# claserken/SISS

Hardware: AMD Instinct MI355X
Metric: unlearning samples/sec (= unlearning-steps/sec x batch x gpus), CelebA-HQ-256 DDPM SISS (higher is better)
Workload: dtype bf16; 1 GPU; delete_celeb.yaml: CelebA-HQ 256x256 DDPM UNet (113.7M params), SISS lambd=0.5, t=999, bf16, bs=16/GPU, GA=1, scaling_norm=500, AdamW lr 5e-6; loss_fn=importance_sampling_with_mixture, global_batch=16, grad_accum=1, parallelism=dp1, hipgraph=True

## Files before the change

### include/siss_hip.h

```cpp
#ifndef SISS_HIP_H
#define SISS_HIP_H
#include <stdint.h>
#ifdef __cplusplus
extern "C" {
#endif

typedef struct siss_tn_job {
    const void* Y; long ldy; const void* X; long ldx; float* dW; long set_stride;
    int N, C, npanels, nsets, rows_per_set, row_begin, row_end, nsplits;
    long x_set_rows;
    const void* zero_page; float* dbias; float* dbias2;
    int shifts[9]; int coffs[9];
    long bias_set_stride;
} siss_tn_job;

typedef struct siss_rk_terms {
    const double* row[8]; double c[8]; int n;
} siss_rk_terms;

long siss_loss_partials_words(int B, long chw);
int siss_mixture_fwd(const void* x0, const void* a0, const void* noise, int in_bf16, const int64_t* t, const
    float* u, const float* alphas_cumprod, const float* gamma_tab, const float* sigma_tab, float lambd, int B,
    long chw, void* x_mix, float* gamma_t, float* sigma_t, float* dist_x, float* dist_a, float* iw_x, float* iw_a,
    double* partials, void* stream);
// ... 18 lines not shown
int siss_dispatch_reset(void);
int siss_gemm_nt_set_c3p_blocks(int n);
int siss_gemm_nt(const void* A, long lda, const void* W, void* C, long ldc, const float* bias, const float*
    rowbias, long ldrb, const void* R, long ldr, int M, int N, int Kp, int npanels, const int* shifts, const int*
    coffs, int rows_per_image, int Hp, int Wp, float alpha, int batch, long strideA, long strideW, long strideC,
    void* stream);
int siss_gemm_nt_alpha_cols(const void* A, long lda, const void* W, void* C, long ldc, const float* bias,
    const void* R, long ldr, int M, int N, int Kp, float alpha, int alpha_cols, void* stream);
int siss_gemm_nt_qstats(const void* A, long lda, const void* W, void* C, long ldc, const float* bias, const
    float* rowbias, long ldrb, const void* R, long ldr, int M, int N, int Kp, int npanels, const int* shifts,
    const int* coffs, int rows_per_image, int Hp, int Wp, float alpha, float* qstats, int* written, void* stream);
int siss_conv3x3_sc_takes(int M, int N, int Kp, int K2, int rows_per_image, int Wp, long lda, long ldc, long
    lda2);
int siss_conv3x3_sc(const void* A, long lda, const void* W, void* C, long ldc, const float* bias, const float*
    rowbias, long ldrb, const void* A2, long lda2, const void* W2, int K2, const float* bias2, int M, int N, int
    Kp, const int* shifts, const int* coffs, int rows_per_image, int Hp, int Wp, float* qstats, int* written,
    void* stream);
int siss_conv3x3_dgrad_sc_takes(int M, int N, int Kp, int Nx, int rows_per_image, int Wp, long lda, long ldc,
    long ldcx, long ldr);
int siss_conv3x3_dgrad_sc(const void* A, long lda, const void* W, void* C, long ldc, const void* R, long ldr,
    const void* Wx, void* Cx, long ldcx, int Nx, int M, int N, int Kp, const int* shifts, const int* coffs, int
    rows_per_image, int Hp, int Wp, void* stream);
int siss_gemm_nt_d2s(const void* A, long lda, const void* W, void* C, long ldc, const void* R, long ldr, int
    M, int N, int Kp, int npanels, const int* shifts, const int* coffs, int rows_per_image, int Hp, int Wp, int
    plane, void* stream);
int siss_gemm_nt_d2s_bias(const void* A, long lda, const void* W, void* C, long ldc, const float* bias, int M,
    int N, int Kp, int npanels, const int* shifts, const int* coffs, int rows_per_image, int Hp, int Wp, int
    plane, void* stream);
int siss_gemm_nt_d2s_phases(const void* A, long lda, const void* W, void* C, long ldc, const float* bias,
    const void* R, long ldr, int M, int N, int Kp, const int* phase_p0, const int* shifts, const int* coffs, int
    rows_per_image, int Hp, int Wp, void* stream);
int siss_gemm_nt_geglu_bwd(const void* A, long lda, const void* W, void* dh, const void* h, long rows_x, int
    M, int N, int Kp, void* stream);
int siss_gemm_nt_geglu_fwd(const void* A, long lda, const void* W, const float* bias, void* h, void* y, int M,
    int F, int Kp, void* stream);
long siss_conv_qstats_words(long M, int N);
int siss_gemm_nt_mulsub(const void* A, long lda, const void* W, void* C, long ldc, const void* R, long ldr,
    const float* rowsub, int M, int N, int Kp, float alpha, int batch, long strideA, long strideW, long strideC,
    void* stream);

int siss_gemm_tn(const void* Y, long ldy, const void* X, long ldx, float* dW, long set_stride, int N, int C,
    int npanels, const int* shifts, const int* coffs, int nsets, int rows_per_set, long x_set_rows, int row_begin,
    int row_end, int nsplits, const void* zero_page, float* dbias, float* dbias2, void* stream);
int siss_gemm_tn_bs(const void* Y, long ldy, const void* X, long ldx, float* dW, long set_stride, int N, int
    C, int npanels, const int* shifts, const int* coffs, int nsets, int rows_per_set, long x_set_rows, int
    row_begin, int row_end, int nsplits, const void* zero_page, float* dbias, float* dbias2, long bias_set_stride,
    void* stream);
long siss_gemm_tn_overwrite_log(long* out, long max_records);
int siss_gemm_tn_set_pair_cost(int permille);
int siss_gemm_tn_pair(const void* job3, const void* job1, int max_blocks, void* stream);
int siss_gemm_tn_grouped(const void* jobs, int njobs, void* stream);
int siss_gemm_tn_grouped_capped(const void* jobs, int njobs, int max_blocks, void* stream);

int siss_groupnorm_set_slab(int on);
long siss_gn_partial_words(int n, int H, int W, int C, int G);
int siss_quad_stats(const void* x, long ld, int M, int N, int rows_per_image, float* qs, void* stream);
int siss_groupnorm_fwd_qs(const void* x, const float* gamma, const float* beta, void* y, float* mean, float*
    rstd, float* partial, const float* qsA, int ca, const float* qsB, int N, int H, int W, int C, int G, float
    eps, int silu, int out_compact, int ldx, void* stream);
int siss_groupnorm_fwd_ld(const void* x, const float* gamma, const float* beta, void* y, float* mean, float*
    rstd, float* partial, int N, int H, int W, int C, int G, float eps, int silu, int out_compact, int ldx, void*
    stream);
int siss_groupnorm_fwd(const void* x, const float* gamma, const float* beta, void* y, float* mean, float*
    rstd, float* partial, int N, int H, int W, int C, int G, float eps, int silu, int out_compact, void* stream);
int siss_groupnorm_bwd_ld(const void* dy, const void* x, const float* gamma, const float* beta, const float*
    mean, const float* rstd, void* dx, const void* accum, const void* accum2, void* dx2, int split_c, int
    accumulate2, float* dgamma, float* dbeta, float* colsum, long colsum_ld, float* partial, int n2, int nx, int
    set_images, long set_stride, int H, int W, int C, int G, int silu, int dy_compact, int ldx, void* stream);
int siss_groupnorm_bwd_ld_s2d(const void* dy, const void* x, const float* gamma, const float* beta, const
    float* mean, const float* rstd, void* dx, const void* accum, const void* accum2, void* dx2, int split_c, int
    accumulate2, float* dgamma, float* dbeta, float* colsum, long colsum_ld, float* partial, int n2, int nx, int
    set_images, long set_stride, int H, int W, int C, int G, int silu, int dy_compact, int ldx, void* stream);
int siss_groupnorm_bwd(const void* dy, const void* x, const float* gamma, const float* beta, const float*
    mean, const float* rstd, void* dx, const void* accum, const void* accum2, void* dx2, int split_c, int
    accumulate2, float* dgamma, float* dbeta, float* colsum, long colsum_ld, float* partial, int n2, int nx, int
    set_images, long set_stride, int H, int W, int C, int G, int silu, int dy_compact, void* stream);
int siss_groupnorm_bwd_sc(const void* dy, const void* x, const float* gamma, const float* beta, const float*
    mean, const float* rstd, void* dx, const void* dout, long ldo, const void* wsc, int K, const void* accum2,
    void* dx2, int split_c, int accumulate2, float* dgamma, float* dbeta, float* colsum, float* partial, float*
    gconst, int n2, int nx, int set_images, long set_stride, int H, int W, int C, int G, int silu, int s2d, int
    ldx, void* stream);

int siss_conv_out_fprop(const void* x, const float* w, const float* bias, float* pred, int B, int H, int W,
    int C, int CO, void* stream);
int siss_conv_out_dgrad(const float* c, const float* w, void* dx, int N2, int H, int W, int C, int CO, void*
    stream);
int siss_conv_out_wgrad(const float* c, const void* x, float* dW, float* dbias, int nsets, int set_images, int
    nx, long set_stride_w, long set_stride_b, int H, int W, int C, int CO, void* stream);
int siss_conv_in_dgrad(const void* dh, long ld, const void* w, int kp, float* dx, int N, int Cin, int H, int
    W, int C0, void* stream);
int siss_conv_in_dgrad_f32(const void* dh, long ld, const void* w, int kp, float* dx, int N, int Cin, int H,
    int W, int C0, void* stream);

int siss_softmax_fwd(const void* s, void* p, long rows, int S, void* stream);
int siss_softmax_bwd(const void* p, const void* dp, void* ds, long rows, long p_rows, int S, float scale,
    void* stream);
int siss_mha_small_takes(int S, int D, int training);
int siss_mha_small_fwd(const void* q, const void* k, const void* v, void* o, float* lse, int N, int S, int C,
    int D, float scale, void* stream);
int siss_mha_small_bwd(const void* q, const void* k, const void* v, const void* o, const float* lse, const
    void* dout, void* dq, void* dk, void* dv, int n2, int nx, int S, int C, int D, float scale, void* stream);
int siss_mha_small_fwd_f32(const void* q, const void* k, const void* v, void* o, float* lse, int N, int S, int
    C, int D, float scale, void* stream);
int siss_mha_small_bwd_f32(const void* q, const void* k, const void* v, const void* o, const float* lse, const
    void* dout, void* dq, void* dk, void* dv, int n2, int nx, int S, int C, int D, float scale, void* stream);

// ... 337 lines not shown
```

### siss_amd/csrc/common.h

```cpp
#pragma once
#include <hip/hip_runtime.h>
#include <stdint.h>

typedef uint16_t bf16_t;

typedef __attribute__((ext_vector_type(8))) short bf16x8_t;
typedef __attribute__((ext_vector_type(4))) float f32x4_t;
typedef __attribute__((ext_vector_type(16))) float f32x16_t;
typedef __attribute__((ext_vector_type(4))) uint32_t u32x4_t;
typedef __attribute__((ext_vector_type(2))) uint32_t u32x2_t;
typedef __attribute__((ext_vector_type(2))) float f32x2_t;
typedef __attribute__((ext_vector_type(2))) __bf16 bf16x2_t;

#define SISS_OK 0
#define SISS_ERR_ARG 1
#define SISS_ERR_LAUNCH 2

#define SISS_CHECK_ARG(cond) \
    do {                     \
        if (!(cond)) return SISS_ERR_ARG; \
    } while (0)

#define SISS_LAUNCH_RET()                                 \
    do {                                                  \
// ... 55 lines not shown
    return __builtin_bit_cast(float, b0) + __builtin_bit_cast(float, b1);
}

__device__ __forceinline__ float sigmoid_f(float z) { return __builtin_amdgcn_rcpf(1.f + __expf(-z)); }
__device__ __forceinline__ float silu_f(float z) { return z * sigmoid_f(z); }
__device__ __forceinline__ float dsilu_f(float z) {
    const float s = sigmoid_f(z);
    return s * (1.f + z * (1.f - s));
}

__device__ __forceinline__ void gelu_parts(float g, float& Phi, float& e) {
    const float x = fabsf(g) * 0.70710678118654752f;
    const float t = __builtin_amdgcn_rcpf(fmaf(0.3275911f, x, 1.f));
    e = __builtin_amdgcn_exp2f(g * g * -0.72134752044448170f);
    const float poly = t * fmaf(t, fmaf(t, fmaf(t, fmaf(t, 1.061405429f, -1.453152027f), 1.421413741f), -0.284496736f), 0.254829592f);
    const float erf_abs = fmaf(-poly, e, 1.f);
    Phi = 0.5f * (1.f + copysignf(erf_abs, g));
}
__device__ __forceinline__ float gelu_f(float g) { float P, e; gelu_parts(g, P, e); return g * P; }
__device__ __forceinline__ float dgelu_f(float g) { float P, e; gelu_parts(g, P, e); return fmaf(g * 0.3989422804014327f, e, P); }


__device__ __forceinline__ void glds16_asm(const void* g, unsigned lds_dst) {
    unsigned keep;
    asm volatile("s_mov_b32 %0, m0\n\ts_mov_b32 m0, %2\n\ts_nop 0\n\tglobal_load_lds_dwordx4 %1, off\n\ts_mov_b32 m0, %0"
                 : "=&s"(keep) : "v"(g), "s"(lds_dst) : "memory");
}
__device__ __forceinline__ void glds16_saddr(unsigned off, const void* base, unsigned lds_dst) {
    asm volatile("s_mov_b32 m0, %1\n\ts_nop 0\n\tglobal_load_lds_dwordx4 %0, %2" :: "v"(off), "s"(lds_dst), "s"(base) : "memory");
}
__device__ __forceinline__ unsigned lds_addr(const void* p) {
    return (unsigned)(size_t)(__attribute__((address_space(3))) const char*)p;
}

static inline int cdiv(long a, long b) { return (int)((a + b - 1) / b); }

constexpr int kMaxDevices = 64;
constexpr int kQsTileRows = 254, kQsHalfRows = 128;
static inline int siss_current_device() {
    int dev = 0;
    return hipGetDevice(&dev) == hipSuccess && dev >= 0 && dev < kMaxDevices ? dev : -1;
}
static inline int siss_ensure_smem(const void* kernel, int bytes, unsigned char (&done)[kMaxDevices]) {
    const int dev = siss_current_device();
    if (dev < 0) return SISS_ERR_LAUNCH;
    if (!__atomic_load_n(&done[dev], __ATOMIC_ACQUIRE)) {
        if (hipFuncSetAttribute(kernel, hipFuncAttributeMaxDynamicSharedMemorySize, bytes) != hipSuccess) return SISS_ERR_LAUNCH;
        __atomic_store_n(&done[dev], (unsigned char)1, __ATOMIC_RELEASE);
    }
    return SISS_OK;
}

enum SissKernelId { SISS_K_NT = 0, SISS_K_NT_C3P, SISS_K_FLASH_FWD, SISS_K_FLASH_BWD, SISS_K_NT_SPLITK, SISS_K_TN1, SISS_K_TN3,
                    SISS_K_GN_SLAB, SISS_K_GN_QSTATS, SISS_K_FLASH_QSPLIT, SISS_K_ATTN1H_FWD, SISS_K_ATTN1H_BWD, SISS_K_TN_PAIR, SISS_K_FLASH32, SISS_K_FLASH32_FWD, SISS_K_NT_WIDE, SISS_K_GN_SC, SISS_K_COUNT };
void siss_count_dispatch(int kernel_id);
void* siss_workspace(long* bytes);
```

### siss_amd/csrc/groupnorm.hip

```cpp
#include "nt_common.h"
#include "gn_host.h"

namespace {

constexpr int kStatsDepth = 2;
constexpr int kThreads = 256;
constexpr int kMaxG = 32;
constexpr int kMaxC = 1024;

struct GNShape {
    int H, W, C, G, cpg, lpp, ppi;
    int chunk_px, nchunks;
    int ld, Gf, nslices;
    int ldx;
};

__device__ __forceinline__ long compact_row(int n, int pi, int H, int W) { return (long)n * H * W + pi; }

__device__ __forceinline__ void unpack8(u32x4_t r, float (&v)[8]) {
#pragma unroll
    for (int j = 0; j < 4; ++j) {
        v[2 * j] = __builtin_bit_cast(float, r[j] << 16);
        v[2 * j + 1] = __builtin_bit_cast(float, r[j] & 0xffff0000u);
    }
// ... 682 lines not shown
            vx[q] = vd[q] = u32x4_t{0u, 0u, 0u, 0u};
            if (EXTRA) vb[q] = vc[q] = u32x4_t{0u, 0u, 0u, 0u};
            if (s2d_lane) {
                const int yy = y - 1, xx = xq - 1;
                dst[q] = p.dx + nc + (((long)(kset * p.nx + img) * img2 + ((yy >> 1) + 1) * wl2 + (xx >> 1) + 1) * 4 + (((yy & 1) << 1) | (xx & 1))) * p.split_c;
            } else {
                dst[q] = obase + (set_row0 + r) * ostride;
            }
            if (state[q] == 2) {
                vx[q] = *reinterpret_cast<const u32x4_t*>(xb + (long)r * p.ldx);
                vd[q] = *reinterpret_cast<const u32x4_t*>(db + (long)r * C);
                if (EXTRA && bb) vb[q] = *reinterpret_cast<const u32x4_t*>(bb + (long)r * C);
                if (EXTRA && oacc) vc[q] = *reinterpret_cast<const u32x4_t*>(dst[q]);
            }
        }
#pragma unroll
        for (int q = 0; q < kBatch; ++q) {
            if (state[q] == 0) continue;
            u32x4_t out = u32x4_t{0u, 0u, 0u, 0u};
            if (state[q] == 2) {
                if (slot_of[q] != cur_slot) { cur_slot = slot_of[q]; load_consts(cur_slot); }
                const int row = (it0 + q) * 16 + trow;
                float v[8], d[8], pr[8], o[8];
                unpack8(vx[q], v);
                unpack8(vd[q], d);
                unpack8(*reinterpret_cast<const u32x4_t*>(smem + row * kCRow + chunk * 16), pr);
#pragma unroll
                for (int e = 0; e < 8; ++e) {
                    float xh, dsl;
                    gn_bwd_xhat<SILU>(v[e], rs[e], mr[e], ga[e], be[e], xh, dsl);
                    o[e] = gn_bwd_t(d[e], dsl, xh, rs[e], m1[e], m2[e]);
                }
#pragma unroll
                for (int e = 0; e < 8; ++e) o[e] += pr[e];
                if (EXTRA && bb) {
                    float r8[8];
                    unpack8(vb[q], r8);
#pragma unroll
                    for (int e = 0; e < 8; ++e) o[e] += r8[e];
                }
                if (EXTRA && any_oacc) {
                    float r8[8];
                    unpack8(vc[q], r8);
#pragma unroll
                    for (int e = 0; e < 8; ++e) o[e] += r8[e];
                }
                out = pack8(o);
            }
            *reinterpret_cast<u32x4_t*>(dst[q]) = out;
        }
    }
}

constexpr int kBlocksFwd = 768, kBlocksBwd = 512, kBlocksBwdStats = 767;

bool make_shape(int H, int W, int C, int G, GNShape& s, int N = 16, int blocks = kBlocksFwd) {
    if (H <= 0 || W <= 0 || C <= 0 || G <= 0 || G > kMaxG || C % G || C % 8) return false;
    s.H = H; s.W = W; s.ld = C; s.ldx = C; s.Gf = G; s.cpg = C / G;
    int gs = G;
    if (C > kMaxC) {
        int best = 0, best_util = -1;
        gs = 0;
        for (int d = G; d >= 1; --d) {
            if (G % d) continue;
            const int cs = d * s.cpg;
            if (cs > kMaxC || cs % 8) continue;
            const int lpp = cs / 8, util = (kThreads / lpp) * lpp;
            if (util * 10 >= kThreads * 9) { gs = d; break; }
            if (util > best_util) { best_util = util; best = d; }
        }
        if (gs == 0) gs = best;
        if (gs == 0) return false;
    }
    s.G = gs; s.C = gs * s.cpg; s.nslices = G / gs;
    s.lpp = s.C / 8;
    if (s.lpp > kThreads) return false;
    s.ppi = kThreads / s.lpp;
    const int px = H * W;
    int nch = (blocks + N * s.nslices - 1) / (N * s.nslices);
    const int max_by_work = (px + 16 * s.ppi - 1) / (16 * s.ppi);
    if (nch > max_by_work) nch = max_by_work;
    if (blocks == kBlocksBwd || blocks == kBlocksBwdStats) {
        const int by_work32 = (px + 32 * s.ppi - 1) / (32 * s.ppi);
        if (nch > by_work32 && (long)by_work32 * N * s.nslices >= 256) nch = by_work32;
    }
    if (nch > 256) nch = 256;
    if (nch < 1) nch = 1;
    s.chunk_px = (px + nch - 1) / nch;
    s.nchunks = (px + s.chunk_px - 1) / s.chunk_px;
    return true;
}

int g_use_slab = 1;

}

extern "C" {

int siss_groupnorm_set_slab(int on) {
    g_use_slab = on != 0;
    return g_use_slab;
}

long siss_gn_partial_words(int n, int H, int W, int C, int G) {
    GNShape s;
    if (!make_shape(H, W, C, G, s, 1)) return -1;
    return (long)n * s.nslices * s.nchunks * 2 * s.G;
}

int siss_quad_stats(const void* x, long ld, int M, int N, int rows_per_image, float* qs, void* stream) {
    SISS_CHECK_ARG(x && qs && M > 0 && N > 0 && N % 8 == 0 && N <= 8 * kThreads && ld >= N && ld % 8 == 0 && rows_per_image >= 256);
    SISS_CHECK_ARG((uintptr_t)x % 16 == 0 && (uintptr_t)qs % 8 == 0 && (N >> 3) * 4 <= kThreads);
    const int tiles = (M + kQsTileRows - 1) / kQsTileRows;
    gn_quad_stats_kernel<<<dim3(2 * tiles), kThreads, 0, (hipStream_t)stream>>>((const bf16_t*)x, ld, M, N, rows_per_image, qs);
    SISS_LAUNCH_RET();
}

int siss_groupnorm_fwd_qs(const void* x, const float* gamma, const float* beta, void* y, float* mean,
                          float* rstd, float* partial, const float* qsA, int ca, const float* qsB, int N, int H, int W,
                          int C, int G, float eps, int silu, int out_compact, int ldx, void* stream) {
    GNShape s;
    SISS_CHECK_ARG(!qsA || (ca > 0 && ca <= C && ca % 4 == 0 && (ca == C) == (qsB == nullptr)));
    SISS_CHECK_ARG(((uintptr_t)qsA | (uintptr_t)qsB) % 8 == 0);
    SISS_CHECK_ARG(x && gamma && beta && y && mean && rstd && partial && N > 0);
    SISS_CHECK_ARG(make_shape(H, W, C, G, s, N, kBlocksFwd));
    SISS_CHECK_ARG(ldx == 0 || (ldx >= C && ldx % 8 == 0));
    if (ldx) s.ldx = ldx;
    SISS_CHECK_ARG(((uintptr_t)x | (uintptr_t)y | (uintptr_t)partial) % 16 == 0);
    if (g_use_slab && s.nslices == 1) {
        const int rc = siss_gn_slab_fwd(x, gamma, beta, y, mean, rstd, N, H, W, C, G, eps, silu, out_compact, ldx, stream);
        if (rc >= 0) return rc;
    }
    hipStream_t st = (hipStream_t)stream;
    dim3 grid(s.nchunks, N, s.nslices);
    if (qsA && s.cpg % 4 == 0 && (long)(H + 2) * (W + 2) >= 256) {
        siss_count_dispatch(SISS_K_GN_QSTATS);
        gn_qstats_finalize_kernel<<<dim3(N, (G + 3) / 4), kThreads, 0, st>>>(qsA, ca / 4, qsB, (C - ca) / 4, H, W, G, s.cpg, eps,
                                                                             mean, rstd);
        partial = nullptr;
    } else
        gn_stats_kernel<<<grid, kThreads, 0, st>>>((const bf16_t*)x, s, partial);
    if (silu)
        gn_apply_kernel<true><<<grid, kThreads, 0, st>>>((const bf16_t*)x, gamma, beta, partial, s, eps, out_compact, (bf16_t*)y, mean, rstd);
    else
        gn_apply_kernel<false><<<grid, kThreads, 0, st>>>((const bf16_t*)x, gamma, beta, partial, s, eps, out_compact, (bf16_t*)y, mean, rstd);
    SISS_LAUNCH_RET();
}
int siss_groupnorm_fwd_ld(const void* x, const float* gamma, const float* beta, void* y, float* mean,
                          float* rstd, float* partial, int N, int H, int W, int C, int G, float eps,
                          int silu, int out_compact, int ldx, void* stream) {
// ... 59 lines not shown
}
int siss_groupnorm_bwd_ld_s2d(const void* dy, const void* x, const float* gamma, const float* beta,
                              const float* mean, const float* rstd, void* dx, const void* accum, const void* accum2,
                              void* dx2, int split_c, int accumulate2, float* dgamma,
                              float* dbeta, float* colsum, long colsum_ld, float* partial, int n2, int nx, int set_images,
                              long set_stride, int H, int W, int C, int G, int silu, int dy_compact, int ldx, void* stream) {
    return gn_bwd_launch(gn_bwd_call(dy, x, gamma, beta, mean, rstd, dx, accum, accum2, dx2, split_c, accumulate2, dgamma, dbeta, colsum,
                                     colsum_ld, partial, n2, nx, set_images, set_stride, H, W, C, G, silu, dy_compact, ldx, stream), 1);
}
int siss_groupnorm_bwd(const void* dy, const void* x, const float* gamma, const float* beta,
                       const float* mean, const float* rstd, void* dx, const void* accum, const void* accum2,
                       void* dx2, int split_c, int accumulate2, float* dgamma,
                       float* dbeta, float* colsum, long colsum_ld, float* partial, int n2, int nx, int set_images,
                       long set_stride, int H, int W, int C, int G, int silu, int dy_compact, void* stream) {
    return siss_groupnorm_bwd_ld(dy, x, gamma, beta, mean, rstd, dx, accum, accum2, dx2, split_c, accumulate2, dgamma, dbeta,
                                 colsum, colsum_ld, partial, n2, nx, set_images, set_stride, H, W, C, G, silu, dy_compact, 0,
                                 stream);
}

int siss_groupnorm_bwd_sc(const void* dy, const void* x, const float* gamma, const float* beta, const float* mean,
                          const float* rstd, void* dx, const void* dout, long ldo, const void* wsc, int K, const void* accum2,
                          void* dx2, int split_c, int accumulate2, float* dgamma, float* dbeta, float* colsum, float* partial,
                          float* gconst, int n2, int nx, int set_images, long set_stride, int H, int W, int C, int G, int silu,
                          int s2d, int ldx, void* stream) {
    GNShape ss;
    SISS_CHECK_ARG(!colsum);
    GNBwdCall c = {};
    c.dy = dy; c.x = x; c.gamma = gamma; c.beta = beta; c.mean = mean; c.rstd = rstd; c.dx = dx; c.accum2 = accum2; c.dx2 = dx2;
    c.split_c = split_c; c.dgamma = dgamma; c.dbeta = dbeta; c.partial = partial; c.n2 = n2; c.nx = nx; c.set_images = set_images;
    c.H = H; c.W = W; c.C = C; c.ldx = ldx;
    if (const int rc = gn_bwd_check(c, s2d)) return rc;
    SISS_CHECK_ARG(dout && wsc && gconst && ((uintptr_t)dout | (uintptr_t)wsc | (uintptr_t)gconst) % 16 == 0);
    SISS_CHECK_ARG(K > 0 && K % BK == 0 && ldo >= K && ldo % 8 == 0);
    SISS_CHECK_ARG(make_shape(H, W, C, G, ss, nx, kBlocksBwdStats) && ss.nslices == 1);
    const long rpi = (long)(H + 2) * (W + 2);
    SISS_CHECK_ARG(rpi >= 64 && nx * rpi < (1L << 31) - 256);
    if (ldx) ss.ldx = ldx;
    hipStream_t st = (hipStream_t)stream;
    static unsigned char attr_set[2][2][2][kMaxDevices];
    const bool extra = accum2 != nullptr || (dx2 && accumulate2);
    const bf16_t* dyp = (const bf16_t*)dy; const bf16_t* xp = (const bf16_t*)x;
    dim3 grid_s(ss.nchunks, nx, 1);
#define GN_SC_STATS(SILU, SETS) \
    gn_bwd_stats_kernel<SILU, SETS><<<grid_s, kThreads, 0, st>>>(dyp, xp, gamma, beta, mean, rstd, ss, nx, 0, set_images, set_stride, partial, dgamma, dbeta)
    if (n2 == nx) { if (silu) { GN_SC_STATS(true, 1); } else { GN_SC_STATS(false, 1); } }
    else          { if (silu) { GN_SC_STATS(true, 2); } else { GN_SC_STATS(false, 2); } }
#undef GN_SC_STATS
    gn_bwd_sc_finalize_kernel<<<n2, kThreads, 0, st>>>(partial, ss.nchunks, mean, rstd, G, nx, (double)H * W * ss.cpg, (f32x4_t*)gconst);
    GNSCParams p;
    p.A = (const bf16_t*)dout; p.Wt = (const bf16_t*)wsc; p.x = xp; p.dy = dyp; p.accum2 = (const bf16_t*)accum2;
    p.gamma = gamma; p.beta = beta; p.gconst = (const f32x4_t*)gconst; p.dx = (bf16_t*)dx; p.dx2 = (bf16_t*)dx2;
    p.lda = ldo; p.ldx = ss.ldx; p.K = K; p.C = C; p.G = G; p.cpg = ss.cpg; p.Mset = (int)(nx * rpi); p.nx = nx; p.sets = n2 / nx;
    p.rpi = (int)rpi; p.H = H; p.W = W; p.split_c = split_c; p.accumulate2 = accumulate2; p.inv_wp = 1.0f / (float)(W + 2);
    const unsigned blocks = (unsigned)(cdiv(p.Mset, 128) * cdiv(C, BN) * p.sets);
#define GN_SC_(SILU, S2D_, EX)                                                                                                \
    do {                                                                                                                      \
        if (siss_ensure_smem((const void*)gn_bwd_sc_kernel<SILU, S2D_, EX>, kScSmemBytes, attr_set[SILU][S2D_][EX]) != SISS_OK) return SISS_ERR_LAUNCH; \
        gn_bwd_sc_kernel<SILU, S2D_, EX><<<blocks, kThreads, kScSmemBytes, st>>>(p);                                           \
    } while (0)
#define GN_SC(SILU, S2D_) do { if (extra) GN_SC_(SILU, S2D_, true); else GN_SC_(SILU, S2D_, false); } while (0)
    if (silu) { if (s2d) GN_SC(true, true); else GN_SC(true, false); }
    else      { if (s2d) GN_SC(false, true); else GN_SC(false, false); }
#undef GN_SC
#undef GN_SC_
    siss_count_dispatch(SISS_K_GN_SC);
    SISS_LAUNCH_RET();
}

}
```

### siss_amd/lib.py

```python
import ctypes as C
import os
import re
import threading

import torch

from . import prof

_HERE = os.path.dirname(os.path.abspath(__file__))
LIB_PATH = os.environ.get("SISS_LIB_PATH") or os.path.join(_HERE, "libsiss_hip.so")

P, I, L, D = C.c_void_p, C.c_int, C.c_long, C.c_double
HEADER = os.path.join(os.path.dirname(_HERE), "include", "siss_hip.h")
_SCALARS = {"int": C.c_int, "long": C.c_long, "float": C.c_float, "double": C.c_double}


def parse_prototypes(text):
    text = " ".join(re.sub(r"/\*.*?\*/", " ", text, flags=re.S).split())
    out = {}
    for ret, name, params in re.findall(r"\b(int|long) (siss_\w+) ?\(([^()]*)\) ?;", text):
        out[name] = (_SCALARS[ret], [])
        for decl in ([] if params.strip() in ("", "void") else params.split(",")):
            m = re.fullmatch(r"(?:const )?(\w+)( ?\* ?| )(\w+)", decl.strip())
            if m and "*" in m.group(2):
# ... 11 lines not shown
PARAMS = {n: tuple(p for _, p in ps) for n, (_, ps) in _PROTOTYPES.items()}
RESTYPE = {n: r for n, (r, _) in _PROTOTYPES.items()}

F32_ENTRY = {n: n + "_f32" for n in (
    "siss_gemm_nt", "siss_gemm_tn", "siss_groupnorm_fwd_ld", "siss_groupnorm_bwd_ld", "siss_upsample2x", "siss_upsample2x_bwd",
    "siss_concat", "siss_concat_tail", "siss_concat_bwd", "siss_add_inplace", "siss_space_to_depth_ld", "siss_depth_to_space",
    "siss_pad_to_compact", "siss_compact_add_to_pad", "siss_im2col3x3", "siss_conv_out_fprop", "siss_mha_small_fwd",
    "siss_mha_small_bwd", "siss_softmax_fwd", "siss_softmax_bwd", "siss_softmax_rows_fwd", "siss_softmax_rows_bwd",
    "siss_layernorm_fwd", "siss_layernorm_bwd", "siss_geglu_fwd", "siss_geglu_bwd", "siss_head_split", "siss_head_merge",
    "siss_rowdot", "siss_gemm_nt_mulsub", "siss_conv_in_dgrad")}
F32_ENTRY.update({"siss_transpose_bf16": "siss_transpose_f32", "siss_cast_f32_bf16": "siss_copy_f32",
                  "siss_conv_weight_dgrad_multi_bf16": "siss_conv_weight_dgrad_multi_f32"})
F32_ENTRY.update({n: n + "_f32" for n in ("siss_gemm_nt_d2s", "siss_gemm_nt_d2s_bias", "siss_gemm_nt_d2s_phases", "siss_conv3x3_sc", "siss_conv3x3_dgrad_sc",
                                          "siss_gemm_tn_bs", "siss_gemm_tn_grouped", "siss_groupnorm_bwd_ld_s2d",
                                          "siss_upsample_phase_weights")})
F32_SAME = {"siss_zero_ranges", "siss_upsample_phase_wgrad_fold", "siss_timestep_sincos", "siss_linear_small_fwd", "siss_linear_small_bwd", "siss_linear_multi_fwd", "siss_linear_multi_bwd",
            "siss_nchw_channel_sums", "siss_mixture_fwd", "siss_mixture_select", "siss_loss_bwd_seed", "siss_mse_bwd_seed",
            "siss_ddpm_step", "siss_cfg_ddim_step", "siss_cfg_dpmpp_step", "siss_pflow_drift_div", "siss_slab_rowsum_f64", "siss_rk_combine", "siss_rk_norm", "siss_pair_noise", "siss_pair_sqerr", "siss_metric_conv", "siss_metric_maxpool3", "siss_inc_avgpool", "siss_inc_global_avg", "siss_inc_preprocess", "siss_fid_stats_update", "siss_kmeans_decoded", "siss_kmeans_finalize", "siss_kmeans_assign", "siss_kmeans_update", "siss_sscd_preprocess", "siss_sscd_gem", "siss_sscd_normalize_score", "siss_clipiqa_avgpool", "siss_clipiqa_token_mean", "siss_clipiqa_fold_query", "siss_clipiqa_scores", "siss_clipiqa_pool", "siss_clipiqa_head_value", "siss_clipiqa_score", "siss_quick_gelu_f32", "siss_grad_norms_scale", "siss_grad_norm_partials", "siss_grad_scalars", "siss_recombine_clip_adamw",
            "siss_grad_norms_scale_ranges", "siss_recombine_clip_adamw_ranges",
            "siss_grad_norm_single", "siss_clip_adamw_ema", "siss_ema_advance", "siss_ema_step", "siss_swap_f32",
            "siss_ctx_dgrad", "siss_ctx_reduce", "siss_noise_norm_cot", "siss_prompt_embed_update", "siss_latent_inject", "siss_latent_sample", "siss_image_gather",
            "siss_lora_project", "siss_lora_merge", "siss_lora_project_conv", "siss_lora_merge_conv",
            "siss_absf_select", "siss_saliency_mask", "siss_grad_norms_scale_masked", "siss_recombine_clip_adamw_masked",
            "siss_fisher_accumulate", "siss_grad_norms_scale_ewc",
            "siss_ssd_ratio", "siss_ssd_dampen",
            "siss_sscd_topk", "siss_sscd_count_above", "siss_sscd_fill_above"}
for _b, _f in F32_ENTRY.items():
    if SIGNATURES[_b] != SIGNATURES[_f]:
        raise TypeError(f"{_f} does not have the argument types of {_b} in {HEADER}")
_MODE = threading.local()


def in_f32_mode():
    return bool(getattr(_MODE, "f32", False))


class f32_mode:

    def __init__(self, on):
        self.on = bool(on)

    def __enter__(self):
        self.prev, _MODE.f32 = getattr(_MODE, "f32", False), self.on
        return self

    def __exit__(self, *exc):
        _MODE.f32 = self.prev
        return False


KERNEL_IDS = {"gemm_nt_kernel": 0, "gemm_nt_c3p_kernel": 1, "flash_attn_fwd": 2, "flash_attn_bwd": 3,
              "gemm_nt_kernel/splitk": 4, "gemm_tn_kernel<1>": 5, "gemm_tn_kernel<3>": 6, "gn_slab": 7, "gn_qstats": 8, "flash_dkdv_qsplit": 9,
              "attn1h_fwd": 10, "attn1h_bwd": 11, "gemm_tn_pair": 12, "flash32_bwd": 13, "flash32_fwd": 14, "gemm_nt_kernel/wide": 15,
              "gn_bwd_sc_kernel": 16}


def dispatch_counts(reset=False):
    lib = load()
    out = {k: int(lib.siss_dispatch_count(i)) for k, i in KERNEL_IDS.items()}
    if reset:
        lib.siss_dispatch_reset()
    return out



class TNJob(C.Structure):
    _fields_ = [("Y", P), ("ldy", L), ("X", P), ("ldx", L), ("dW", P), ("set_stride", L),
                ("N", I), ("C", I), ("npanels", I), ("nsets", I), ("rows_per_set", I), ("row_begin", I), ("row_end", I),
                ("nsplits", I), ("x_set_rows", L), ("zero_page", P), ("dbias", P), ("dbias2", P),
                ("shifts", I * 9), ("coffs", I * 9), ("bias_set_stride", L)]


class RkTerms(C.Structure):
    _fields_ = [("row", P * 8), ("c", D * 8), ("n", I)]

    @classmethod
    def of(cls, pairs):
        pairs = list(pairs)
        assert len(pairs) <= 8
        t = cls()
        for j, (c, r) in enumerate(pairs):
            assert r.dtype == torch.float64 and r.is_cuda and r.is_contiguous()
            t.row[j], t.c[j] = r.data_ptr(), float(c)
        t.n = len(pairs)
        return t


_lib = None
MIN_ABI = 5


def load():
    global _lib
    if _lib is not None:
        return _lib
    if not os.path.exists(LIB_PATH):
        raise RuntimeError(
            f"{LIB_PATH} not found: build it with `python -m siss_amd.build` "
            "(there is no CPU fallback for the SISS hot path)")
    lib = C.CDLL(LIB_PATH)
    override = os.path.abspath(LIB_PATH) != os.path.join(_HERE, "libsiss_hip.so")
    for name, argtypes in SIGNATURES.items():
        try:
            fn = getattr(lib, name)
        except AttributeError:
            if override:
                continue
# ... 99 lines not shown
```

Before: 309.3 samples/sec.

## Add persistent walking variant of fused GroupNorm-backward shortcut GEMM kernel

Adds a persistent kernel for small-K shortcut GEMMs fused with GroupNorm backward. Each block keeps its weight fragments in registers and walks several M tiles, prefetching the next A tile while it applies the current epilogue, with XCD-aware tile assignment. This removes the per-tile weight reload and launch-granularity overhead of the one-tile-per-block kernel. It adds a tunable block count, higher register and shared-memory use, and more complex wait-count logic, and it only applies when K/BK is at most 2.

Result: no change. 311.8 samples/sec, median of 6 (+0.8%).

```diff
diff --git a/include/siss_hip.h b/include/siss_hip.h
--- a/include/siss_hip.h
+++ b/include/siss_hip.h
@@ -94,6 +94,7 @@
 int siss_gemm_tn_grouped(const void* jobs, int njobs, void* stream);
 int siss_gemm_tn_grouped_capped(const void* jobs, int njobs, int max_blocks, void* stream);
 
+int siss_groupnorm_bwd_sc_set_blocks(int n);
 int siss_groupnorm_set_slab(int on);
 long siss_gn_partial_words(int n, int H, int W, int C, int G);
 int siss_quad_stats(const void* x, long ld, int M, int N, int rows_per_image, float* qs, void* stream);
diff --git a/siss_amd/csrc/common.h b/siss_amd/csrc/common.h
--- a/siss_amd/csrc/common.h
+++ b/siss_amd/csrc/common.h
@@ -131,6 +131,6 @@
 }
 
 enum SissKernelId { SISS_K_NT = 0, SISS_K_NT_C3P, SISS_K_FLASH_FWD, SISS_K_FLASH_BWD, SISS_K_NT_SPLITK, SISS_K_TN1, SISS_K_TN3,
-                    SISS_K_GN_SLAB, SISS_K_GN_QSTATS, SISS_K_FLASH_QSPLIT, SISS_K_ATTN1H_FWD, SISS_K_ATTN1H_BWD, SISS_K_TN_PAIR, SISS_K_FLASH32, SISS_K_FLASH32_FWD, SISS_K_NT_WIDE, SISS_K_GN_SC, SISS_K_COUNT };
+                    SISS_K_GN_SLAB, SISS_K_GN_QSTATS, SISS_K_FLASH_QSPLIT, SISS_K_ATTN1H_FWD, SISS_K_ATTN1H_BWD, SISS_K_TN_PAIR, SISS_K_FLASH32, SISS_K_FLASH32_FWD, SISS_K_NT_WIDE, SISS_K_GN_SC, SISS_K_GN_SC_WALK, SISS_K_COUNT };
 void siss_count_dispatch(int kernel_id);
 void* siss_workspace(long* bytes);
diff --git a/siss_amd/csrc/groupnorm.hip b/siss_amd/csrc/groupnorm.hip
--- a/siss_amd/csrc/groupnorm.hip
+++ b/siss_amd/csrc/groupnorm.hip
@@ -758,6 +758,274 @@
     }
 }
 
+constexpr int kScWalkMaxSteps = 2;
+constexpr int kScWalkSlab = 128 * 128;
+constexpr int sc_walk_smem(int ks) { return ks * kScWalkSlab + kScTileBytes + 3 * kMaxG * 16 + 2 * BN * 4; }
+static_assert(kScWalkMaxSteps * kScWalkSlab <= kScTileBytes, "W is staged through the tile buffer");
+static_assert(2 * sc_walk_smem(kScWalkMaxSteps) <= 160 * 1024, "two blocks per CU");
+
+template <int N> __device__ __forceinline__ void wait_vm_upto(int n) {
+    if constexpr (N == 0) { asm volatile("s_waitcnt vmcnt(0)" ::: "memory"); }
+    else {
+        if (n >= N) asm volatile("s_waitcnt vmcnt(%0)" :: "n"(N) : "memory");
+        else wait_vm_upto<N - 1>(n);
+    }
+}
+
+template <bool SILU, bool S2D, bool EXTRA, int KS>
+__global__ __launch_bounds__(kThreads, 2) void gn_bwd_sc_walk_kernel(const GNSCParams p, const int groups) {
+    constexpr int BM = 128, kPieces = BM / 8 / 4, kABytes = KS * kScWalkSlab;
+    extern __shared__ __attribute__((aligned(16))) char smem[];
+    char* const tile = smem + kABytes;
+    f32x4_t* const cst = reinterpret_cast<f32x4_t*>(tile + kScTileBytes);
+    float* const gb = reinterpret_cast<float*>(cst + 3 * kMaxG);
+    const int tid = threadIdx.x, lane = tid & 63;
+    const int w = __builtin_amdgcn_readfirstlane(tid >> 6);
+    const int tiles_n = (p.C + BN - 1) / BN, tiles_m = (p.Mset + BM - 1) / BM;
+    const int combos = tiles_n * p.sets;
+    int k, t0, t1, tstep;
+    if ((groups & 7) == 0) {
+        const int xcd = blockIdx.x & 7, q = tiles_m >> 3, r = tiles_m & 7;
+        k = blockIdx.x >> 3;
+        const int start = xcd < r ? xcd * (q + 1) : r * (q + 1) + (xcd - r) * q;
+        tstep = groups >> 3; t0 = start + k / combos; t1 = start + q + (xcd < r ? 1 : 0);
+    } else {
+        k = blockIdx.x; tstep = groups; t0 = k / combos; t1 = tiles_m;
+    }
+    if (t0 >= t1) return;
+    const int combo = k % combos;
+    const int tn = combo % tiles_n, kset = combo / tiles_n;
+    const int n0 = tn * BN;
+    const long set_row0 = (long)kset * p.Mset;
+    const bf16_t* const A = p.A + set_row0 * p.lda;
+    const unsigned smem_a = lds_addr(smem), tile_a = smem_a + kABytes;
+
+    auto issue_a = [&](int m0) {
+#pragma unroll
+        for (int j = 0; j < kPieces; ++j) {
+            const int row = (w * kPieces + j) * 8 + (lane >> 3);
+            const int lc = (lane & 7) ^ ((row >> 1) & 7);
+            const int last = p.Mset - 1 - m0;
+            const unsigned off = ((unsigned)(row < last ? row : last) * (unsigned)p.lda + lc * 8) * 2;
+            const bf16_t* base = A + (long)m0 * p.lda;
+#pragma unroll
+            for (int s = 0; s < KS; ++s) glds16_saddr(off + s * BK * 2, base, smem_a + s * kScWalkSlab + (w * kPieces + j) * 1024);
+        }
+    };
+#pragma unroll
+    for (int j = 0; j < kPieces; ++j) {
+        const int row = (w * kPieces + j) * 8 + (lane >> 3);
+        const int lc = (lane & 7) ^ ((row >> 1) & 7);
+        int gn = n0 + row; gn = gn < p.C ? gn : p.C - 1;
+        const bf16_t* src = p.Wt + (long)gn * p.K + lc * 8;
+#pragma unroll
+        for (int s = 0; s < KS; ++s) glds16_asm(src + s * BK, tile_a + s * kScWalkSlab + (w * kPieces + j) * 1024);
+    }
+    issue_a(t0 * BM);
+    const int chunk = tid & 15, trow = tid >> 4;
+    const int nc = n0 + chunk * 8;
+    const bool cols = nc < p.C;
+    if (tid < 2 * BN) {
+        const int c = n0 + (tid & (BN - 1));
+        gb[tid] = c < p.C ? (tid < BN ? p.gamma[c] : p.beta[c]) : 0.f;
+    }
+    float ga[8], be[8];
+    const int frow = lane & 15, fq = lane >> 4;
+    const int a_off0 = frow * 128 + ((fq ^ ((frow >> 1) & 7)) << 4);
+    asm volatile("s_waitcnt vmcnt(0)" ::: "memory");
+    __builtin_amdgcn_s_barrier();
+    bf16x8_t wf[KS][2][2];
+#pragma unroll
+    for (int s = 0; s < KS; ++s)
+#pragma unroll
+        for (int kk = 0; kk < 2; ++kk)
+#pragma unroll
+            for (int i = 0; i < 2; ++i) {
+                const int rw = w * 32 + i * 16 + frow;
+                const int off = s * kScWalkSlab + rw * 128 + ((fq ^ ((rw >> 1) & 7)) << 4);
+                wf[s][kk][i] = *reinterpret_cast<const bf16x8_t*>(tile + (off ^ (kk << 6)));
+            }
+
+    const int rpi = p.rpi;
+    const int g0 = nc / p.cpg, rem0 = nc - g0 * p.cpg;
+    float rs[8], mr[8], m1[8], m2[8];
+    auto load_consts = [&](int slot) {
+        const f32x4_t* c = cst + slot * p.G;
+        int g = g0, rm = rem0;
+#pragma unroll
+        for (int e = 0; e < 8; ++e) {
+            const f32x4_t v = c[g];
+            rs[e] = v[0]; mr[e] = v[1]; m1[e] = v[2]; m2[e] = v[3];
+            if (++rm == p.cpg) { rm = 0; ++g; }
+        }
+    };
+#pragma unroll
+    for (int e = 0; e < 8; ++e) rs[e] = mr[e] = m1[e] = m2[e] = 0.f;
+    int cst_img0 = -1;
+    int cur_img = -1;
+    const int Wp = p.W + 2, Hp = p.H + 2;
+    const int C = p.C;
+    const bool second = p.dx2 != nullptr && nc >= p.split_c;
+    const int ostride = p.dx2 ? (second ? C - p.split_c : p.split_c) : C;
+    const bool oacc = EXTRA && second && p.accumulate2;
+    const bool any_oacc = EXTRA && p.dx2 != nullptr && p.accumulate2;
+    const bool s2d_lane = S2D && !second;
+    bf16_t* const obase = second ? p.dx2 + (nc - p.split_c) : p.dx + nc;
+    const int wl2 = (p.W >> 1) + 2;
+    const long img2 = (long)((p.H >> 1) + 2) * wl2;
+    const bool has_b = EXTRA && p.accum2 != nullptr;
+    const unsigned lb = cols ? (unsigned)nc * 2 : 0u, xrb = (unsigned)p.ldx * 2, drb = (unsigned)C * 2;
+    constexpr int kBatch = EXTRA ? 2 : 4;
+    int nst = 0;
+
+    for (int tm = t0; tm < t1; tm += tstep) {
+        const int m0 = tm * BM;
+        const int img0 = m0 / rpi;
+        const int b1 = (img0 + 1) * rpi - m0, b2 = b1 + rpi;
+        const bf16_t* const xt = p.x + (long)m0 * p.ldx;
+        const bf16_t* const dt = p.dy + (set_row0 + m0) * C;
+        const bf16_t* const bt = has_b ? p.accum2 + (set_row0 + m0) * C : nullptr;
+        const int last_row = p.Mset - 1 - m0;
+        auto geom = [&](int row, int& img, int& y, int& xq) {
+            img = img0 + (row >= b1) + (row >= b2);
+            const int rem = m0 + row - img * rpi;
+            y = (int)(((float)rem + 0.5f) * p.inv_wp); xq = rem - y * Wp;
+        };
+        auto dst_of = [&](int row, int img, int y, int xq) -> bf16_t* {
+            if (s2d_lane) {
+                const int yy = y - 1, xx = xq - 1;
+                return p.dx + nc + (((long)(kset * p.nx + img) * img2 + ((yy >> 1) + 1) * wl2 + (xx >> 1) + 1) * 4 + (((yy & 1) << 1) | (xx & 1))) * p.split_c;
+            }
+            return obase + (set_row0 + m0 + row) * ostride;
+        };
+        u32x4_t vx[kBatch], vd[kBatch], vb[EXTRA ? kBatch : 1], vc[EXTRA ? kBatch : 1];
+        int state[kBatch];
+        auto load_rows = [&](int it0) {
+#pragma unroll
+            for (int q = 0; q < kBatch; ++q) {
+                const int row = (it0 + q) * 16 + trow;
+                int img, y, xq;
+                geom(row, img, y, xq);
+                const bool halo = (y == 0) | (y == Hp - 1) | (xq == 0) | (xq == Wp - 1);
+                state[q] = (!cols || row > last_row) ? 0 : (halo ? (s2d_lane ? 0 : 1) : 2);
+                const int rowc = row < last_row ? row : last_row;
+                vx[q] = ld16(xt, boff(rowc, xrb, lb));
+                vd[q] = ld16(dt, boff(rowc, drb, lb));
+                if (EXTRA) {
+                    vb[q] = vc[q] = u32x4_t{0u, 0u, 0u, 0u};
+                    if (has_b) vb[q] = ld16(bt, boff(rowc, drb, lb));
+                    if (oacc && state[q] == 2) vc[q] = *reinterpret_cast<const u32x4_t*>(dst_of(row, img, y, xq));
+                }
+            }
+        };
+        auto apply_rows = [&](int it0) {
+            nst = 0;
+#pragma unroll
+            for (int q = 0; q < kBatch; ++q) nst += __builtin_amdgcn_ballot_w64(state[q] != 0) != 0 ? 1 : 0;
+            u32x4_t out[kBatch];
+#pragma unroll
+            for (int q = 0; q < kBatch; ++q) {
+                const int row = (it0 + q) * 16 + trow;
+                if (state[q] == 2) {
+                    const int img = img0 + (row >= b1) + (row >= b2);
+                    if (img != cur_img) { cur_img = img; load_consts(cur_img - img0); }
+                }
+                float v[8], d[8], pr[8], o[8];
+                unpack8(vx[q], v);
+                unpack8(vd[q], d);
+                unpack8(*reinterpret_cast<const u32x4_t*>(tile + row * kCRow + chunk * 16), pr);
+#pragma unroll
+                for (int e = 0; e < 8; ++e) {
+                    float xh, dsl;
+                    gn_bwd_xhat<SILU>(v[e], rs[e], mr[e], ga[e], be[e], xh, dsl);
+                    o[e] = gn_bwd_t(d[e], dsl, xh, rs[e], m1[e], m2[e]);
+                }
+#pragma unroll
+                for (int e = 0; e < 8; ++e) o[e] += pr[e];
+                if (EXTRA && has_b) {
+                    float r8[8];
+                    unpack8(vb[q], r8);
+#pragma unroll
+                    for (int e = 0; e < 8; ++e) o[e] += r8[e];
+                }
+                if (EXTRA && any_oacc) {
+                    float r8[8];
+                    unpack8(vc[q], r8);
+#pragma unroll
+                    for (int e = 0; e < 8; ++e) o[e] += r8[e];
+                }
+                out[q] = pack8(o);
+                asm volatile("" : "+v"(out[q][0]), "+v"(out[q][1]), "+v"(out[q][2]), "+v"(out[q][3]));
+            }
+#pragma unroll
+            for (int q = 0; q < kBatch; ++q) {
+                if (state[q] == 0) continue;
+                const int row = (it0 + q) * 16 + trow;
+                int img, y, xq;
+                geom(row, img, y, xq);
+                *reinterpret_cast<u32x4_t*>(dst_of(row, img, y, xq)) = state[q] == 2 ? out[q] : u32x4_t{0u, 0u, 0u, 0u};
+            }
+        };
+
+        wait_vm_upto<kBatch>(__builtin_amdgcn_readfirstlane(nst));
+        asm volatile("s_waitcnt lgkmcnt(0)" ::: "memory");
+        __builtin_amdgcn_s_barrier();
+        if (img0 != cst_img0) {
+            if (tid < 3 * p.G) {
+                const int slot = tid / p.G, g = tid - slot * p.G;
+                int img = img0 + slot; img = img < p.nx ? img : p.nx - 1;
+                cst[tid] = p.gconst[(long)(kset * p.nx + img) * p.G + g];
+            }
+            cst_img0 = img0;
+        }
+        load_rows(0);
+        f32x4_t acc[2][8];
+#pragma unroll
+        for (int i = 0; i < 2; ++i)
+#pragma unroll
+            for (int j = 0; j < 8; ++j) acc[i][j] = f32x4_t{0.f, 0.f, 0.f, 0.f};
+#pragma unroll
+        for (int s = 0; s < KS; ++s)
+#pragma unroll
+            for (int kk = 0; kk < 2; ++kk) {
+                bf16x8_t af[8];
+#pragma unroll
+                for (int j = 0; j < 8; ++j) af[j] = *reinterpret_cast<const bf16x8_t*>(smem + s * kScWalkSlab + j * 2048 + (a_off0 ^ (kk << 6)));
+#pragma unroll
+                for (int i = 0; i < 2; ++i)
+#pragma unroll
+                    for (int j = 0; j < 8; ++j)
+                        acc[i][j] = __builtin_amdgcn_mfma_f32_16x16x32_bf16(wf[s][kk][i], af[j], acc[i][j], 0, 0, 0);
+            }
+#pragma unroll
+        for (int j = 0; j < 8; ++j) {
+            const int m = j * 16 + frow;
+#pragma unroll
+            for (int i = 0; i < 2; ++i) {
+                const int nl = w * 32 + i * 16 + fq * 4;
+                const f32x4_t v = acc[i][j];
+                *reinterpret_cast<u32x2_t*>(tile + m * kCRow + nl * 2) = u32x2_t{pack_bf2(v[0], v[1]), pack_bf2(v[2], v[3])};
+            }
+        }
+        asm volatile("s_waitcnt lgkmcnt(0)" ::: "memory");
+        __builtin_amdgcn_s_barrier();
+        cur_img = -1;
+#pragma unroll
+        for (int e = 0; e < 8; e += 4) {
+            const f32x4_t gv = *reinterpret_cast<const f32x4_t*>(gb + chunk * 8 + e), bv = *reinterpret_cast<const f32x4_t*>(gb + BN + chunk * 8 + e);
+#pragma unroll
+            for (int r = 0; r < 4; ++r) { ga[e + r] = gv[r]; be[e + r] = bv[r]; }
+        }
+        apply_rows(0);
+        if (tm + tstep < t1) issue_a(m0 + tstep * BM);
+#pragma unroll 1
+        for (int it0 = kBatch; it0 < BM / 16; it0 += kBatch) {
+            load_rows(it0);
+            apply_rows(it0);
+        }
+    }
+}
+
 constexpr int kBlocksFwd = 768, kBlocksBwd = 512, kBlocksBwdStats = 767;
 
 bool make_shape(int H, int W, int C, int G, GNShape& s, int N = 16, int blocks = kBlocksFwd) {
@@ -799,9 +1067,20 @@
 
 int g_use_slab = 1;
 
+constexpr int kScWalkBlocks = 512;
+int g_sc_blocks[kMaxDevices];
+
 }
 
 extern "C" {
+
+int siss_groupnorm_bwd_sc_set_blocks(int n) {
+    if (n < 0 || n > 2048) return -1;
+    const int dev = siss_current_device();
+    if (dev < 0) return -1;
+    g_sc_blocks[dev] = n;
+    return n ? n : kScWalkBlocks;
+}
 
 int siss_groupnorm_set_slab(int on) {
     g_use_slab = on != 0;
@@ -967,8 +1246,35 @@
     p.gamma = gamma; p.beta = beta; p.gconst = (const f32x4_t*)gconst; p.dx = (bf16_t*)dx; p.dx2 = (bf16_t*)dx2;
     p.lda = ldo; p.ldx = ss.ldx; p.K = K; p.C = C; p.G = G; p.cpg = ss.cpg; p.Mset = (int)(nx * rpi); p.nx = nx; p.sets = n2 / nx;
     p.rpi = (int)rpi; p.H = H; p.W = W; p.split_c = split_c; p.accumulate2 = accumulate2; p.inv_wp = 1.0f / (float)(W + 2);
+    if (K / BK <= kScWalkMaxSteps) {
+        const int tiles_m = cdiv(p.Mset, 128), combos = cdiv(C, BN) * p.sets;
+        const int dev = siss_current_device();
+        if (dev < 0) return SISS_ERR_LAUNCH;
+        int groups = (g_sc_blocks[dev] ? g_sc_blocks[dev] : kScWalkBlocks) / combos;
+        if (groups > ((tiles_m + 7) & ~7)) groups = (tiles_m + 7) & ~7;
+        if (groups >= 8) groups &= ~7;
+        if (groups < 1) groups = 1;
+        const unsigned wblocks = (unsigned)(groups * combos);
+        const int ks = K / BK, wsmem = sc_walk_smem(ks);
+        static unsigned char wattr_set[2][2][2][kScWalkMaxSteps][kMaxDevices];
+#define GN_SCW_(SILU, S2D_, EX, KS_)                                                                                          \
+    do {                                                                                                                      \
+        if (siss_ensure_smem((const void*)gn_bwd_sc_walk_kernel<SILU, S2D_, EX, KS_>, wsmem, wattr_set[SILU][S2D_][EX][KS_ - 1]) != SISS_OK) return SISS_ERR_LAUNCH; \
+        gn_bwd_sc_walk_kernel<SILU, S2D_, EX, KS_><<<wblocks, kThreads, wsmem, st>>>(p, groups);                               \
+    } while (0)
+#define GN_SCW(SILU, S2D_, EX) do { if (ks == 1) GN_SCW_(SILU, S2D_, EX, 1); else GN_SCW_(SILU, S2D_, EX, 2); } while (0)
+#define GN_SCW2(SILU, S2D_) do { if (extra) GN_SCW(SILU, S2D_, true); else GN_SCW(SILU, S2D_, false); } while (0)
+        if (silu) { if (s2d) GN_SCW2(true, true); else GN_SCW2(true, false); }
+        else      { if (s2d) GN_SCW2(false, true); else GN_SCW2(false, false); }
+#undef GN_SCW2
+#undef GN_SCW
+#undef GN_SCW_
+        siss_count_dispatch(SISS_K_GN_SC);
+        siss_count_dispatch(SISS_K_GN_SC_WALK);
+        SISS_LAUNCH_RET();
+    }
     const unsigned blocks = (unsigned)(cdiv(p.Mset, 128) * cdiv(C, BN) * p.sets);
-#define GN_SC_(SILU, S2D_, EX)                                                                                                \
+#define GN_SC_(SILU, S2D_, EX)                                                                                              \
     do {                                                                                                                      \
         if (siss_ensure_smem((const void*)gn_bwd_sc_kernel<SILU, S2D_, EX>, kScSmemBytes, attr_set[SILU][S2D_][EX]) != SISS_OK) return SISS_ERR_LAUNCH; \
         gn_bwd_sc_kernel<SILU, S2D_, EX><<<blocks, kThreads, kScSmemBytes, st>>>(p);                                           \
diff --git a/siss_amd/lib.py b/siss_amd/lib.py
--- a/siss_amd/lib.py
+++ b/siss_amd/lib.py
@@ -87,7 +87,7 @@
 KERNEL_IDS = {"gemm_nt_kernel": 0, "gemm_nt_c3p_kernel": 1, "flash_attn_fwd": 2, "flash_attn_bwd": 3,
               "gemm_nt_kernel/splitk": 4, "gemm_tn_kernel<1>": 5, "gemm_tn_kernel<3>": 6, "gn_slab": 7, "gn_qstats": 8, "flash_dkdv_qsplit": 9,
               "attn1h_fwd": 10, "attn1h_bwd": 11, "gemm_tn_pair": 12, "flash32_bwd": 13, "flash32_fwd": 14, "gemm_nt_kernel/wide": 15,
-              "gn_bwd_sc_kernel": 16}
+              "gn_bwd_sc_kernel": 16, "gn_bwd_sc_kernel/walk": 17}
 
 
 def dispatch_counts(reset=False):
```
